# ThomasHelfer/multimodal-supernovae

Measured on AMD Instinct MI355X. Metric: contrastive pairs/sec (image+light-curve) at global batch 1024, 1/2/4/8 GPUs, higher is better.
Workload: dtype f32; 1 GPU; ViT-S/8 image tower (64x64x3, build-defined) + reference light-curve transformer (T=200, emb 64, 8 heads, depth 5, 2 bands) -> enc_dim 128, symmetric InfoNCE with all-gathered global negatives, RAdam; full train step; per_gpu_batch=1024, global_batch=1024, parallelism=dp1, launch=eager, gemm_precision=bf16x6

## Files before the change

### include/msn_hip.h

```cpp
#ifndef MSN_HIP_H
#define MSN_HIP_H

#include <stddef.h>
#include <stdint.h>

#ifdef __cplusplus
extern "C" {
#endif

#define MSN_OK 0
#define MSN_ERR_SHAPE 1
#define MSN_ERR_HIP 2

typedef void* msn_stream_t;

int msn_version(void);
const char* msn_last_error(void);
int msn_clock_probe(unsigned long long* out2, int microseconds, msn_stream_t stream);
int msn_device_count(void);

#define MSN_OP_N 0
#define MSN_OP_T 1
#define MSN_EPI_NONE 0
#define MSN_EPI_RELU 1
// ... 100 lines not shown

size_t msn_plane_bytes(int64_t R, int64_t C, int planes);
size_t msn_plane_split_colsum_workspace_bytes(int64_t R, int64_t C);
int msn_plane_split(const float* x, int64_t ldx, int64_t R, int64_t C, int planes, int transposed, void* out, float* colsum,
                    void* ws, size_t ws_bytes, msn_stream_t stream);
typedef struct msn_split_item {
    const float* x;
    int64_t ldx, R, C;
    int transposed;
    void* out;
} msn_split_item;
int msn_plane_split_list(int n, const msn_split_item* items, int planes, msn_stream_t stream);
int msn_plane_merge(const void* planes_in, int planes, int64_t R, int64_t C, float* y, int64_t ldy, msn_stream_t stream);
size_t msn_pgemm_nt_colsum_workspace_bytes(int64_t M, int N);
size_t msn_pgemm_nt_workspace_bytes(int64_t M, int N, int K, int planes, int c_planes, int epilogue, int want_colsum);
int msn_set_pgemm_tail_split(int enabled);
int msn_pgemm_nt(int64_t M, int N, int K, int planes, const void* A, const void* B, void* C, int64_t ldc, int c_planes,
                 const float* bias, int epilogue, float* aux, int64_t ldaux, float* colsum_out, void* ws, size_t ws_bytes,
                 msn_stream_t stream);
size_t msn_pgemm_tn_workspace_bytes(int64_t M, int N, int K, int planes);
int msn_pgemm_tn(int64_t M, int N, int K, int planes, const void* A, const void* B, float* C, int64_t ldc, void* ws,
                 size_t ws_bytes, msn_stream_t stream);
int msn_layernorm_fwd_planes(const float* x, int64_t ldx, int64_t rows, int cols, const float* gamma, const float* beta,
                             float eps, int planes, void* y_planes, float* y, int64_t ldy, float* mean, float* rstd,
                             msn_stream_t stream);
int msn_layernorm_bwd_planes(const float* dy, int64_t lddy, const float* x, int64_t ldx, int64_t rows, int cols,
                             const float* mean, const float* rstd, const float* gamma, const float* add, int64_t ldadd,
                             float* dx, int64_t lddx, int planes, void* dx_planes, float* dgamma, float* dbeta,
                             float* dx_colsum, void* ws, size_t ws_bytes, msn_stream_t stream);
int msn_attention_fwd_planes(const float* qkv, int64_t ldqkv, const uint8_t* key_mask, int B, int H, int T, int head_dim,
                             float scale, float* out, int64_t ldo, float* lse, int planes, void* out_planes, msn_stream_t stream);
// ... 204 lines not shown
```

### multimodal_supernovae_amd/_lib.py

```python
import ctypes
import os

import torch

_HERE = os.path.dirname(os.path.abspath(__file__))
LIB_PATH = os.environ.get("MSN_HIP_LIB") or os.path.join(_HERE, "lib", "libmsn_hip.so")

c_i64 = ctypes.c_int64
c_int = ctypes.c_int
c_f32 = ctypes.c_float
c_f64 = ctypes.c_double
c_ptr = ctypes.c_void_p
c_size = ctypes.c_size_t

SIGNATURES = {
    "msn_version": (c_int, []),
    "msn_last_error": (ctypes.c_char_p, []),
    "msn_clock_probe": (c_int, [c_ptr, c_int, c_ptr]),
    "msn_ffn_supported": (c_int, [c_i64, c_int, c_int]),
    "msn_ffn_fwd": (c_int, [c_ptr, c_i64, c_i64, c_int, c_int, c_ptr, c_ptr, c_ptr, c_ptr, c_ptr, c_i64, c_ptr]),
    "msn_ffn_bwd_workspace_bytes": (c_size, [c_i64, c_int, c_int]),
    "msn_ffn_bwd": (c_int, [c_ptr, c_i64, c_ptr, c_i64, c_i64, c_int, c_int, c_ptr, c_ptr, c_ptr, c_ptr, c_i64, c_ptr, c_ptr, c_ptr,
                            c_ptr, c_ptr, c_size, c_ptr]),
    "msn_cls_attention_supported": (c_int, [c_int, c_int]),
# ... 33 lines not shown
    "msn_masked_pool_bwd": (c_int, [c_ptr, c_ptr, c_i64, c_int, c_int, c_int, c_ptr, c_ptr, c_ptr, c_ptr]),
    "msn_mask_tokens": (c_int, [c_ptr, c_ptr, c_i64, c_int, c_ptr, c_ptr]),
    "msn_add_rows": (c_int, [c_ptr, c_i64, c_ptr, c_i64, c_i64, c_int, c_ptr]),
    "msn_plane_bytes": (c_size, [c_i64, c_i64, c_int]),
    "msn_plane_split_colsum_workspace_bytes": (c_size, [c_i64, c_i64]),
    "msn_plane_split": (c_int, [c_ptr, c_i64, c_i64, c_i64, c_int, c_int, c_ptr, c_ptr, c_ptr, c_size, c_ptr]),
    "msn_plane_split_list": (c_int, [c_int, c_ptr, c_int, c_ptr]),
    "msn_plane_split_f16": (c_int, [c_ptr, c_i64, c_i64, c_i64, c_int, c_ptr, c_ptr, c_int, c_ptr, c_ptr, c_size, c_ptr]),
    "msn_pgemm_nt_f16": (c_int, [c_i64, c_int, c_int, c_ptr, c_ptr, c_ptr, c_ptr, c_ptr, c_i64, c_ptr, c_int, c_ptr, c_i64, c_ptr,
                                 c_ptr, c_size, c_ptr]),
    "msn_pgemm_tn_f16": (c_int, [c_i64, c_int, c_int, c_ptr, c_ptr, c_ptr, c_ptr, c_ptr, c_i64, c_ptr, c_size, c_ptr]),
    "msn_plane_merge": (c_int, [c_ptr, c_int, c_i64, c_i64, c_ptr, c_i64, c_ptr]),
    "msn_pgemm_nt_colsum_workspace_bytes": (c_size, [c_i64, c_int]),
    "msn_pgemm_nt_workspace_bytes": (c_size, [c_i64, c_int, c_int, c_int, c_int, c_int, c_int]),
    "msn_set_pgemm_tail_split": (c_int, [c_int]),
    "msn_pgemm_nt": (c_int, [c_i64, c_int, c_int, c_int, c_ptr, c_ptr, c_ptr, c_i64, c_int, c_ptr, c_int, c_ptr, c_i64, c_ptr,
                             c_ptr, c_size, c_ptr]),
    "msn_pgemm_tn_workspace_bytes": (c_size, [c_i64, c_int, c_int, c_int]),
    "msn_pgemm_tn": (c_int, [c_i64, c_int, c_int, c_int, c_ptr, c_ptr, c_ptr, c_i64, c_ptr, c_size, c_ptr]),
    "msn_layernorm_fwd_planes": (c_int, [c_ptr, c_i64, c_i64, c_int, c_ptr, c_ptr, c_f32, c_int, c_ptr, c_ptr, c_i64, c_ptr, c_ptr,
                                         c_ptr]),
    "msn_layernorm_bwd_planes": (c_int, [c_ptr, c_i64, c_ptr, c_i64, c_i64, c_int, c_ptr, c_ptr, c_ptr, c_ptr, c_i64, c_ptr,
                                         c_i64, c_int, c_ptr, c_ptr, c_ptr, c_ptr, c_ptr, c_size, c_ptr]),
    "msn_bgemm_nt": (c_int, [c_i64, c_int, c_int, c_ptr, c_i64, c_ptr, c_i64, c_ptr, c_i64, c_int, c_ptr, c_int, c_ptr, c_i64,
                             c_ptr, c_ptr, c_size, c_ptr]),
    "msn_bgemm_nt_colsum_workspace_bytes": (c_size, [c_i64, c_int]),
    "msn_bgemm_tn_workspace_bytes": (c_size, [c_i64, c_int, c_int]),
    "msn_bgemm_tn": (c_int, [c_i64, c_int, c_int, c_ptr, c_i64, c_ptr, c_i64, c_ptr, c_i64, c_ptr, c_size, c_ptr]),
    "msn_cast_bf16": (c_int, [c_ptr, c_i64, c_ptr, c_ptr]),
    "msn_attention_bf16_fwd": (c_int, [c_ptr, c_i64, c_int, c_int, c_int, c_f32, c_ptr, c_i64, c_ptr, c_ptr]),
# ... 119 lines not shown
            fn.restype = res
            fn.argtypes = args
        _lib = handle
    return _lib


def require_gpu():
    if not torch.cuda.is_available():
        raise MsnHipError("multimodal_supernovae_amd needs an MI355X (gfx950): torch.cuda.is_available() is "
                          "False and the hot path has no CPU implementation")


def check(rc, what=""):
    if rc != 0:
        msg = lib().msn_last_error().decode("utf-8", "replace")
        if rc == 2 and torch.cuda.is_available() and what.startswith(("msn_sgemm", "msn_wgrad", "msn_conv2d")):
            try:
                lib().msn_reset_gemm_counters(stream_ptr())
            except Exception:
                pass
        raise MsnHipError(f"{what or 'libmsn_hip'} failed (code {rc}): {msg}")


def stream_ptr():
    return ctypes.c_void_p(torch.cuda.current_stream().cuda_stream)


def ptr(t):
    return ctypes.c_void_p(t.data_ptr()) if t is not None else ctypes.c_void_p(0)
```

### multimodal_supernovae_amd/csrc/pgemm.hip

```cpp


#include "pgemm_kernels.h"

namespace msn {
extern template __global__ void pgemm_nt_kernel<2, 128, true, false, 2, 4, false>(const PgemmArgs);
extern template __global__ void pgemm_nt_kernel<2, 128, false, false, 2, 4, false>(const PgemmArgs);
extern template __global__ void pgemm_nt_kernel<2, 128, false, true, 4, 2, false, true>(const PgemmArgs);
extern template __global__ void pgemm_tn_kernel<2, 128, true, false, 2, 4>(const PgemmArgs);
extern template __global__ void pgemm_tn_kernel<2, 128, false, false, 2, 4>(const PgemmArgs);
extern template __global__ void pgemm_tn_kernel<2, 128, true, true, 2, 4, true>(const PgemmArgs);
extern template __global__ void pgemm_tn_kernel<2, 128, false, true, 2, 4, true>(const PgemmArgs);
}

namespace msn {

__global__ __launch_bounds__(256) void pgemm_tail_finish_kernel(const PgemmArgs p, int bn) {
    const int tiles_tail = p.tiles_m * p.tiles_n - p.tail_full;
    const int per_tile = BM * bn / 4;
    const int64_t i = (int64_t)blockIdx.x * 256 + threadIdx.x;
    if (i >= (int64_t)tiles_tail * per_tile) return;
    const int tt = (int)(i / per_tile), e = (int)(i % per_tile);
    int tm, tn;
    nt_locate(p, p.tail_full + tt, tm, tn);
    const int row = e / (bn / 4), c4 = e % (bn / 4);
    const int64_t m = (int64_t)tm * BM + row;
    const int n = tn * bn + 4 * c4;
    if (m >= p.M || n >= p.N) return;
    float4 s = make_float4(0.f, 0.f, 0.f, 0.f);
    for (int g = 0; g < p.tail_segs; ++g) {
        const float4 v = *reinterpret_cast<const float4*>(p.tail_slabs + ((int64_t)(tt * p.tail_segs + g) * BM + row) * bn + 4 * c4);
        s.x += v.x; s.y += v.y; s.z += v.z; s.w += v.w;
    }
    if (p.bias) {
        const float4 b = *reinterpret_cast<const float4*>(p.bias + n);
        s.x += b.x; s.y += b.y; s.z += b.z; s.w += b.w;
    }
    if (p.epi == MSN_EPI_ADD) {
        const float4 a = *reinterpret_cast<const float4*>(p.aux + m * p.ldaux + n);
        s.x += a.x; s.y += a.y; s.z += a.z; s.w += a.w;
    } else if (p.epi == MSN_EPI_RELU) {
        s.x = fmaxf(s.x, 0.f); s.y = fmaxf(s.y, 0.f); s.z = fmaxf(s.z, 0.f); s.w = fmaxf(s.w, 0.f);
    }
    *reinterpret_cast<float4*>(static_cast<float*>(p.C) + m * p.ldc + n) = s;
}

__global__ void slab_sum_kernel(const float* __restrict__ slabs, int splits, int64_t n4, int K4, int64_t ldc4,
                                      float* __restrict__ C) {
    for (int64_t i = (int64_t)blockIdx.x * blockDim.x + threadIdx.x; i < n4; i += (int64_t)gridDim.x * blockDim.x) {
        float4 s = make_float4(0.f, 0.f, 0.f, 0.f);
        for (int k0 = 0; k0 < splits; k0 += 8) {
// ... 372 lines not shown
extern "C" int msn_plane_merge(const void* planes_in, int planes, int64_t R, int64_t C, float* y, int64_t ldy, msn_stream_t stream) {
    MSN_REQUIRE(planes_in && y && R > 0 && C > 0 && ldy >= C && planes >= 1 && planes <= 3, "msn_plane_merge: bad operand");
    const int64_t n = R * C;
    hipLaunchKernelGGL(plane_merge_kernel, dim3((unsigned)std::min<int64_t>(cdiv(n, 256), 8192)), dim3(256), 0,
                       static_cast<hipStream_t>(stream), static_cast<const unsigned char*>(planes_in), planes, R, (int)C,
                       2 * (int)cdiv(C, 32), y, ldy);
    MSN_LAUNCH_CHECK();
    return MSN_OK;
}

extern "C" size_t msn_pgemm_nt_colsum_workspace_bytes(int64_t M, int N) {
    if (M <= 0 || N <= 0) return 0;
    return sizeof(float) * (4 * (size_t)cdiv(M, BM) + COLSUM_SLICES) * (size_t)N;
}

namespace {
struct NtTail { int full, segs, steps; };
static int g_pgemm_tail = 1;
NtTail nt_tail_plan(int64_t M, int N, int K, int c_planes, int epilogue, bool want_colsum) {
    NtTail t = {0, 0, 0};
    if (!g_pgemm_tail || c_planes || want_colsum) return t;
    if (epilogue != MSN_EPI_NONE && epilogue != MSN_EPI_RELU && epilogue != MSN_EPI_ADD) return t;
    const int total = (int)(cdiv(M, BM) * cdiv(N, 128)), G = 256;
    const int nk = 2 * (int)cdiv(K, 32);
    if (total <= G / 2) {
        if (nk < 24) return t;
        int segs = std::min(std::min(G / total, nk / 4), 8);
        if (segs < 2) return t;
        t.steps = 2 * (int)cdiv(nk, 2 * segs);
        t.segs = (int)cdiv(nk, t.steps);
        t.full = 0;
        if (t.segs < 2) t = {0, 0, 0};
        return t;
    }
    if (total <= G) return t;
    const int left = total % G;
    if (left == 0 || left > G / 2 || nk < 48) return t;
    int segs = std::min(std::min(G / left, nk / 2), 16);
    if (segs < 2) return t;
    t.steps = 2 * (int)cdiv(nk, 2 * segs);
    t.segs = (int)cdiv(nk, t.steps);
    t.full = total - left;
    if (t.segs < 2) t = {0, 0, 0};
    return t;
}
}
extern "C" int msn_set_pgemm_tail_split(int enabled) {
    g_pgemm_tail = enabled ? 1 : 0;
    return MSN_OK;
}

extern "C" size_t msn_pgemm_nt_workspace_bytes(int64_t M, int N, int K, int planes, int c_planes, int epilogue, int want_colsum) {
    if (M <= 0 || N <= 0 || K <= 0) return 0;
    if (want_colsum) return std::max(msn_pgemm_nt_colsum_workspace_bytes(M, N), msn_colsum_workspace_bytes(M, N));
    const NtTail t = nt_tail_plan(M, N, K, c_planes, epilogue, false);
    const int total = (int)(cdiv(M, BM) * cdiv(N, 128));
    return t.segs ? sizeof(float) * (size_t)(total - t.full) * t.segs * BM * 128 : 0;
}

template <int NP, int BN, bool DUAL, int WM = 2, int WN = 4, bool STAG = false>
static void launch_nt(const PgemmArgs& a, bool outp, int grid, hipStream_t st) {
    if (outp) hipLaunchKernelGGL((pgemm_nt_kernel<NP, BN, true, DUAL, WM, WN, STAG>), dim3((unsigned)grid), dim3(64 * WM * WN), 0, st, a);
    else hipLaunchKernelGGL((pgemm_nt_kernel<NP, BN, false, DUAL, WM, WN, STAG>), dim3((unsigned)grid), dim3(64 * WM * WN), 0, st, a);
}

static int pgemm_nt_impl(int64_t M, int N, int K, int planes, const void* A, const void* B, void* C, int64_t ldc,
                         int c_planes, const float* bias, int epilogue, float* aux, int64_t ldaux, float* colsum_out,
                         void* ws, size_t ws_bytes, msn_stream_t stream, const float* scaleA, const float* scaleB) {
    const bool f16 = scaleA != nullptr;
    MSN_REQUIRE(M > 0 && N > 0 && K > 0 && A && B && C, "msn_pgemm_nt: empty operand");
    MSN_REQUIRE(!f16 || (scaleB && planes == 2 && !c_planes), "msn_pgemm_nt_f16: two fp16 planes per operand, both scales, fp32 result");
    MSN_REQUIRE(planes == 2 || planes == 3, "msn_pgemm_nt: planes must be 2 or 3 (got %d)", planes);
// ... 14 lines not shown
    a.cbA = a.cbB = 2 * (int)cdiv(K, 32);
    a.cbC = 2 * (int)cdiv(N, 32);
    a.epi = epilogue;
    const int bn = 128;
    a.tiles_m = (int)cdiv(M, BM); a.tiles_n = (int)cdiv(N, bn);
    a.super_rows = (int)std::max<int64_t>(1, std::min<int64_t>(8, (2 << 20) / ((int64_t)BM * K * 2 * planes)));
    a.chunk_steps = 0;
    {
        const int cs = 32;
        if ((planes == 3 || f16) && !c_planes && a.cbA > std::max(cs, 48)) {
            const int nch = (int)cdiv(a.cbA, cs);
            a.chunk_steps = 2 * (int)cdiv(a.cbA, 2 * nch);
        }
    }
    a.scaleA = scaleA, a.scaleB = scaleB;
    const NtTail tail = nt_tail_plan(M, N, K, c_planes, epilogue, colsum_out != nullptr);
    if (tail.segs && ws && ws_bytes >= msn_pgemm_nt_workspace_bytes(M, N, K, planes, c_planes, epilogue, 0) && aligned16(ws)) {
        a.tail_full = tail.full; a.tail_segs = tail.segs; a.tail_steps = tail.steps;
        a.tail_slabs = static_cast<float*>(ws);
    }
    a.colpart = nullptr;
    const bool colsum_after = colsum_out && a.chunk_steps > 0;
    if (colsum_out && !colsum_after) {
        const size_t need = msn_pgemm_nt_colsum_workspace_bytes(M, N);
        MSN_REQUIRE(ws && ws_bytes >= need && aligned16(ws), "msn_pgemm_nt: column-sum workspace %zu < %zu bytes", ws_bytes, need);
        a.colpart = static_cast<float*>(ws);
    }
    const int total = a.tiles_m * a.tiles_n;
    const int grid = a.tail_segs ? std::max(a.tail_full ? 256 : 0, (total - a.tail_full) * a.tail_segs) : std::min(total, 256);
    hipStream_t st = static_cast<hipStream_t>(stream);
    if (planes == 3) {
        a.colsum_rows = 4;
        launch_nt<3, 128, true, 4, 2>(a, c_planes != 0, grid, st);
    } else if (f16) {
        a.colsum_rows = 4;
        hipLaunchKernelGGL((pgemm_nt_kernel<2, 128, false, true, 4, 2, false, true>), dim3((unsigned)grid), dim3(512), 0, st, a);
    } else {
        launch_nt<2, 128, false>(a, c_planes != 0, grid, st);
    }
    MSN_LAUNCH_CHECK();
    if (a.tail_segs) {
        const int64_t threads = (int64_t)(total - a.tail_full) * (BM * bn / 4);
        hipLaunchKernelGGL(pgemm_tail_finish_kernel, dim3((unsigned)cdiv(threads, 256)), dim3(256), 0, st, a, bn);
        MSN_LAUNCH_CHECK();
    }
    if (colsum_after) return msn_colsum(static_cast<const float*>(C), ldc, M, N, colsum_out, ws, ws_bytes, stream);
    if (colsum_out) {
        if (colsum_finish(a.colpart, (a.colsum_rows ? a.colsum_rows : 2) * a.tiles_m, N, colsum_out, st) != MSN_OK) {
            set_error("msn_pgemm_nt: column-sum launch failed");
            return MSN_ERR_HIP;
        }
    }
    return MSN_OK;
}

extern "C" int msn_pgemm_nt(int64_t M, int N, int K, int planes, const void* A, const void* B, void* C, int64_t ldc,
                            int c_planes, const float* bias, int epilogue, float* aux, int64_t ldaux, float* colsum_out,
                            void* ws, size_t ws_bytes, msn_stream_t stream) {
// ... 90 lines not shown
```

### multimodal_supernovae_amd/csrc/pgemm_kernels.h

```cpp
#pragma once
#include <algorithm>
#include <type_traits>
#include "msn_common.h"

namespace msn {

typedef _Float16 f16x8 __attribute__((ext_vector_type(8)));
typedef unsigned u32x4 __attribute__((ext_vector_type(4)));
typedef unsigned u32x2 __attribute__((ext_vector_type(2)));
typedef __attribute__((address_space(1))) const void gptr_t;
typedef __attribute__((address_space(3))) void lptr_t;

#ifndef MSN_PG_ST_AUX
#define MSN_PG_ST_AUX 0
#endif
constexpr int BM = 256;

struct PgemmArgs {
    const unsigned char* A;
    const unsigned char* B;
    void* C;
    float* aux;
    const float* bias;
    int64_t ldc, ldaux;
    int64_t M;
    int N, K;
    int rbA, rbB;
    int cbA, cbB;
    int cbC;
    int tiles_m, tiles_n, super_rows, epi;
    int colsum_rows;
    int chunk_steps;
    int tail_full;
    int tail_segs, tail_steps;
    float* tail_slabs;
    float* colpart;
    int splits;
    int rb_per_split;
    float* slabs;
    const float* scaleA;
    const float* scaleB;
};

template <int I, int N, class F>
__device__ __forceinline__ void static_for(F&& f) {
    if constexpr (I < N) {
        f(std::integral_constant<int, I>{});
        static_for<I + 1, N>(f);
    }
}
// ... 300 lines not shown
        wait_lgkm<0>();
        wait_vm(p_was_live ? (NSLOT - 3) * ppw + (STAG ? ppw : Q_BEFORE) : 0);
#ifndef MSN_ABL_PG_NOBAR
        __builtin_amdgcn_s_barrier();
#endif
        __builtin_amdgcn_sched_barrier(0);
        if (!last) req_first(fa[(QA + NP) & 1], fb0[PAR ^ 1], nxt);
        __builtin_amdgcn_sched_barrier(0);
        mult(fa[(QA + NP - 1) & 1], fb0[PAR], SML{});
        issue_chunk(std::integral_constant<int, NG - 1>{});
        __builtin_amdgcn_sched_barrier(0);
        advance();
        c_slot = n_slot;
    };

    int eln = lane;
    int frow_e = 0, fhalf_e = 0, srow = 0, schunk = 0;
    unsigned stg = 0, st_mem = 0;
    auto epi_lane = [&]() {
        asm volatile("" : "+v"(eln));
        frow_e = eln & 31, fhalf_e = eln >> 5;
        srow = eln >> 3, schunk = eln & 7;
        stg = lds0 + (unsigned)(NSLOT * SLOT + wave * STG);
        st_mem = stg + (unsigned)(srow * 128 + ((schunk ^ srow) * 16));
    };
    auto erow = [&](int) { return frow_e; };
    auto ecolq = [&](int b) { return 2 * b + fhalf_e; };
    auto acc_addr = [&](int b) { return stg + (unsigned)(erow(b) * 128 + ((ecolq(b) ^ (erow(b) & 7)) * 16)); };
    auto lds_w128 = [&](unsigned addr, const float (&v)[4]) {
        asm volatile("ds_write_b128 %0, %1\n\ts_nop 1" ::"v"(addr), "v"(*reinterpret_cast<const f32x4*>(v)) : "memory");
// ... 26 lines not shown
    };
    auto stage_chunk = [&](int b, const float (&w)[4]) { lds_w128(acc_addr(b), w); };
    auto tile_flush = [&](rsrc_t rs, int64_t ld, int r0, int n0, auto final_) {
        constexpr int AUX = decltype(final_)::value ? MSN_PG_ST_AUX : 0;
        f32x4 r[4];
#pragma unroll
        for (int q = 0; q < 4; ++q) lds_r128(r[q], st_mem + q * 1024);
        asm volatile("s_waitcnt lgkmcnt(0)" : "+v"(r[0]), "+v"(r[1]), "+v"(r[2]), "+v"(r[3])::"memory");
        __builtin_amdgcn_sched_barrier(0);
        const int n = n0 + 4 * schunk;
        const unsigned lo = n < p.N ? (unsigned)((srow * (int)ld + n) * 4) : OOB;
#pragma unroll
        for (int q = 0; q < 4; ++q)
            __builtin_amdgcn_raw_buffer_store_b128(__builtin_bit_cast(u32x4, r[q]), rs, (int)(lo + (unsigned)((r0 + 8 * q) * (int)ld * 4)), 0, AUX);
    };
    auto slab_flush = [&](rsrc_t rs, int r0, int c0) {
        f32x4 r[4];
#pragma unroll
        for (int q = 0; q < 4; ++q) lds_r128(r[q], st_mem + q * 1024);
        asm volatile("s_waitcnt lgkmcnt(0)" : "+v"(r[0]), "+v"(r[1]), "+v"(r[2]), "+v"(r[3])::"memory");
        __builtin_amdgcn_sched_barrier(0);
#pragma unroll
        for (int q = 0; q < 4; ++q)
            __builtin_amdgcn_raw_buffer_store_b128(__builtin_bit_cast(u32x4, r[q]), rs, ((r0 + 8 * q + srow) * BN + c0 + 4 * schunk) * 4, 0, 0);
    };
    auto store_tile_epi = [&](int tm, int tn, auto epi_, auto mode_) {
        constexpr int epi = decltype(epi_)::value;
        constexpr int MODE = decltype(mode_)::value & 3;
        constexpr bool CS = (decltype(mode_)::value & 4) != 0;
        constexpr bool SLAB = (decltype(mode_)::value & 8) != 0;
        constexpr bool PARTIAL = MODE >= 2, ADDC = (MODE == 1 || MODE == 3) && !OUTP;
        constexpr bool AUXIN = !PARTIAL && (epi == MSN_EPI_RELU_BWD || epi == MSN_EPI_GELU_BWD || epi == MSN_EPI_ADD);
        epi_lane();
        if constexpr (DUAL) {
#pragma unroll
            for (int i = 0; i < MT; ++i)
#pragma unroll
                for (int j = 0; j < NT; ++j) acc[i][j] += acc2[i][j];
        }
        if constexpr (F16) {
            const float os = p.scaleA[0] * p.scaleB[0];
#pragma unroll
            for (int i = 0; i < MT; ++i)
#pragma unroll
                for (int j = 0; j < NT; ++j) acc[i][j] *= os;
        }
        constexpr bool PRE = ADDC || AUXIN;
        constexpr int PW = (MT * NT < 2) ? MT * NT : ((DUAL && !OUTP) ? MT * NT : 1);
        f32x4 pre[PRE ? PW : 1][4];
        const rsrc_t rsC = OUTP ? uniform_rsrc(static_cast<unsigned char*>(p.C) + (int64_t)tm * ARB * p.cbC * (NP * PBLK),
                                               min(max(p.rbA - tm * ARB, 0), ARB) * (int64_t)p.cbC * (NP * PBLK))
                                : rows_rsrc(static_cast<const float*>(p.C), p.ldc, tm);
        const rsrc_t rsAux = rows_rsrc(p.aux, p.ldaux, tm);
        const rsrc_t rsBias = uniform_rsrc(p.bias, p.bias ? p.N * 4 : 0);
        const rsrc_t pre_rs = ADDC ? rsC : rsAux;
        const int64_t pre_ld = ADDC ? p.ldc : p.ldaux;
// ... 2 lines not shown
            if constexpr (PRE && t < MT * NT)
                tile_fetch(pre_rs, pre_ld, wm * (32 * MT) + 32 * (t % MT), tn * BN + wn * (32 * NT) + 32 * (t / MT), pre[t % PW]);
        };
        static_for<0, PW>([&](auto t_) { pre_fetch(t_); });
        static_for<0, NT>([&](auto j_) {
            constexpr int j = decltype(j_)::value;
            const int n0 = tn * BN + wn * (32 * NT) + 32 * j;
            float cs[CS ? 16 : 1];
#pragma unroll
            for (int e = 0; e < (CS ? 16 : 1); ++e) cs[e] = 0.f;
            static_for<0, MT>([&](auto i_) {
                constexpr int i = decltype(i_)::value;
                constexpr int t = j * MT + i;
                const int64_t m0 = (int64_t)tm * BM + wm * (32 * MT) + 32 * i;
                const int rbk = tm * ARB + wm * MT + i;
                const bool live = SLAB || (n0 < p.N && (OUTP ? rbk < p.rbA : m0 < p.M));
                if (!live) {
                    pre_fetch(std::integral_constant<int, t + PW>{});
                    return;
                }
                const bool row_ok = m0 + frow_e < p.M;
                float v[16];
#pragma unroll
                for (int e = 0; e < 16; ++e) v[e] = acc[i][j][e];
                if constexpr (ADDC) {
                    float c0[16];
                    tile_take(pre[t % PW], c0);
                    pre_fetch(std::integral_constant<int, t + PW>{});
#pragma unroll
                    for (int e = 0; e < 16; ++e) v[e] += c0[e];
                }
// ... 79 lines not shown
#ifndef MSN_ABL_PG_NOPSTORE
#pragma unroll
                    for (int q = 0; q < 2 * NP; ++q)
                        if (n0 + 16 * (q / NP) < 16 * p.cbC)
                            __builtin_amdgcn_raw_buffer_store_b128(__builtin_bit_cast(u32x4, img[q]), rsC, blk + q * PBLK, 0, MSN_PG_ST_AUX);
#else
                    asm volatile("" ::"v"(img[0]), "v"(img[1]), "v"(img[2]), "v"(img[3]));
                    (void)blk;
#endif
                } else {
#pragma unroll
                    for (int b = 0; b < 4; ++b) {
                        const float w[4] = {v[4 * b], v[4 * b + 1], v[4 * b + 2], v[4 * b + 3]};
                        stage_chunk(b, w);
                    }
                    if constexpr (SLAB)
                        slab_flush(uniform_rsrc(p.tail_slabs + (int64_t)blockIdx.x * (BM * BN), BM * BN * 4), wm * (32 * MT) + 32 * i,
                                   wn * (32 * NT) + 32 * j);
                    else
                        tile_flush(rsC, p.ldc, wm * (32 * MT) + 32 * i, n0, std::integral_constant<bool, !PARTIAL>{});
                }
                if constexpr (CS) {
#pragma unroll
                    for (int e = 0; e < 16; ++e) cs[e] += v[e];
                }
            });
            if constexpr (CS) {
#pragma unroll
                for (int e = 0; e < 16; ++e) {
                    float t = cs[e];
#pragma unroll
                    for (int o = 1; o < 32; o <<= 1) t += __shfl_xor(t, o, 64);
                    cs[e] = t;
                }
                if (frow_e == 0) {
#pragma unroll
                    for (int b = 0; b < 4; ++b) {
                        const int n = n0 + 8 * b + 4 * fhalf_e;
                        if (n < p.N)
                            *reinterpret_cast<float4*>(p.colpart + (int64_t)(WM * tm + wm) * p.N + n) =
                                make_float4(cs[4 * b], cs[4 * b + 1], cs[4 * b + 2], cs[4 * b + 3]);
                    }
                }
            }
        });
    };
    auto store_tile = [&](int tm, int tn, auto mode_) {
        switch (p.epi) {
            case MSN_EPI_RELU: store_tile_epi(tm, tn, std::integral_constant<int, MSN_EPI_RELU>{}, mode_); break;
            case MSN_EPI_GELU: store_tile_epi(tm, tn, std::integral_constant<int, MSN_EPI_GELU>{}, mode_); break;
            case MSN_EPI_RELU_BWD: store_tile_epi(tm, tn, std::integral_constant<int, MSN_EPI_RELU_BWD>{}, mode_); break;
            case MSN_EPI_GELU_BWD: store_tile_epi(tm, tn, std::integral_constant<int, MSN_EPI_GELU_BWD>{}, mode_); break;
            case MSN_EPI_ADD: store_tile_epi(tm, tn, std::integral_constant<int, MSN_EPI_ADD>{}, mode_); break;
            default: store_tile_epi(tm, tn, std::integral_constant<int, MSN_EPI_NONE>{}, mode_); break;
        }
    };
    auto zero_acc = [&]() {
#pragma unroll
        for (int i = 0; i < MT; ++i)
#pragma unroll
            for (int j = 0; j < NT; ++j)
#pragma unroll
                for (int e = 0; e < 16; ++e) {
                    acc[i][j][e] = 0.f;
                    if constexpr (DUAL) acc2[i][j][e] = 0.f;
                }
    };

#pragma unroll
    for (int s = 0; s < NSLOT - 1; ++s) {
        if (p_live) {
#pragma unroll
            for (int q = 0; q < MAXQ; ++q) issue_q(q);
        }
        advance();
    }
    asm volatile("s_waitcnt vmcnt(0)" ::: "memory");
    __builtin_amdgcn_s_barrier();
    __builtin_amdgcn_sched_barrier(0);
    req_first_settled(0u);

    using T0 = std::integral_constant<int, 0>;
    using T1 = std::integral_constant<int, 1>;
    int tm, tn;
    const int csteps = (!OUTP && p.chunk_steps > 0) ? p.chunk_steps : nk;
    int kb, ke;
    for (int idx = 0; seg_of(idx, tm, tn, kb, ke); ++idx) {
        zero_acc();
        if (ke - kb < nk) {
            for (int k = kb; k < ke; k += 2) {
                step(T0{});
                step(T1{}, k + 2 >= ke);
            }
            wait_lgkm<0>();
            store_tile_epi(tm, tn, std::integral_constant<int, MSN_EPI_NONE>{}, std::integral_constant<int, 2 + 8>{});
            req_first_settled((unsigned)(c_slot * SLOT));
            continue;
        }
        int k0 = 0;
        for (; k0 + csteps < nk; k0 += csteps) {
            for (int k = 0; k < csteps; k += 2) {
                step(T0{});
                step(T1{}, k + 2 >= csteps);
            }
            wait_lgkm<0>();
            if (k0 == 0) store_tile_epi(tm, tn, std::integral_constant<int, MSN_EPI_NONE>{}, std::integral_constant<int, 2>{});
            else store_tile_epi(tm, tn, std::integral_constant<int, MSN_EPI_NONE>{}, std::integral_constant<int, 3>{});
            zero_acc();
            req_first_settled((unsigned)(c_slot * SLOT));
        }
        for (int k = k0; k < nk; k += 2) {
            step(T0{});
            step(T1{}, k + 2 >= nk);
        }
        wait_lgkm<0>();
        if (k0 != 0) store_tile(tm, tn, std::integral_constant<int, 1>{});
        else if (p.colpart) store_tile(tm, tn, std::integral_constant<int, 4>{});
        else store_tile(tm, tn, std::integral_constant<int, 0>{});
        req_first_settled((unsigned)(c_slot * SLOT));
    }
}

template <int NP, int BQ, bool SWAP, bool DUAL, int WM = 2, int WN = 4, bool F16 = false, int FOLDN = 1>
__global__ __launch_bounds__(512, 2) void pgemm_tn_kernel(const PgemmArgs p) {
    static_assert(WM * WN == 8, "eight waves");
    constexpr int PHB = 16 * NP, QHB = (BQ / 16) * NP;
    constexpr int PIECES = (PHB + QHB) / 2;
    constexpr int PP = PHB / 2;
    constexpr int SLOT = PIECES * PBLK;
    constexpr int NSLOT = (4 * SLOT <= 160 * 1024) ? 4 : 3;
    constexpr int MAXQ = (PIECES + 7) / 8;
    constexpr int MT = 8 / WM, NT = BQ / (32 * WN);
    constexpr int NG = NP * (NP + 1) / 2;
    __shared__ __attribute__((aligned(1024))) unsigned char lds[NSLOT * SLOT];
// ... 298 lines not shown
```

### multimodal_supernovae_amd/ops.py

```python
import ctypes
import os

import torch

from . import _lib
from ._lib import check, lib, ptr, stream_ptr

GEMM_PROFILE = None
ATTN_PROFILE = None

PREC_F32, PREC_BF16X3, PREC_BF16 = 0, 1, 2
PREC_PLANES3, PREC_PLANES2 = 3, 4
_PREC_NAMES = {"f32": PREC_F32, "bf16x3": PREC_BF16X3, "bf16": PREC_BF16, "bf16x6": PREC_PLANES3, "bf16x3p": PREC_PLANES2}
_C_PRECISION = {PREC_F32: PREC_F32, PREC_BF16X3: PREC_BF16X3, PREC_BF16: PREC_BF16, PREC_PLANES3: PREC_F32,
                PREC_PLANES2: PREC_BF16X3}


def plane_count(precision=None):
    p = GEMM_PRECISION if precision is None else precision
    return 3 if p == PREC_PLANES3 else 2 if p == PREC_PLANES2 else 0
GEMM_PRECISION = _PREC_NAMES[os.environ.get("MSN_GEMM_PRECISION", "bf16x6").lower()]


class gemm_precision:
# ... 1094 lines not shown
        else:
            check(L.msn_pgemm_tn(M, N, K, dy.planes, ptr(dy.buf), ptr(x.buf), ptr(c), K, ptr(ws), nb, stream_ptr()), "msn_pgemm_tn")
    return c


def layernorm_fwd_planes(x, gamma, beta, eps, planes):
    return _layernorm_fwd(x, gamma, beta, eps, planes=planes)


def layernorm_bwd_planes(dy, x, mean, rstd, gamma, planes, add=None, want_colsum=False):
    out = _layernorm_bwd(dy, x, mean, rstd, gamma, add, want_colsum, planes=planes)
    return out if want_colsum else out[:4]


def set_pgemm_tail_split(enabled):
    check(lib().msn_set_pgemm_tail_split(int(bool(enabled))))
```

Measured before the change: 15610 pairs/s.

## Finish split-K tail tiles in-kernel via atomic arrival counters and widen tail eligibility

```diff
diff --git a/include/msn_hip.h b/include/msn_hip.h
--- a/include/msn_hip.h
+++ b/include/msn_hip.h
@@ -138,7 +138,9 @@
 int msn_plane_merge(const void* planes_in, int planes, int64_t R, int64_t C, float* y, int64_t ldy, msn_stream_t stream);
 size_t msn_pgemm_nt_colsum_workspace_bytes(int64_t M, int N);
 size_t msn_pgemm_nt_workspace_bytes(int64_t M, int N, int K, int planes, int c_planes, int epilogue, int want_colsum);
-int msn_set_pgemm_tail_split(int enabled);
+int msn_set_pgemm_tail_split(int mode);
+int msn_set_pgemm_tail_plan(int max_segs, int min_steps);
+int msn_pgemm_nt_tail_plan(int64_t M, int N, int K, int planes, int c_planes, int epilogue, int want_colsum, int* out3);
 int msn_pgemm_nt(int64_t M, int N, int K, int planes, const void* A, const void* B, void* C, int64_t ldc, int c_planes,
                  const float* bias, int epilogue, float* aux, int64_t ldaux, float* colsum_out, void* ws, size_t ws_bytes,
                  msn_stream_t stream);
diff --git a/multimodal_supernovae_amd/_lib.py b/multimodal_supernovae_amd/_lib.py
--- a/multimodal_supernovae_amd/_lib.py
+++ b/multimodal_supernovae_amd/_lib.py
@@ -71,6 +71,8 @@
     "msn_pgemm_nt_colsum_workspace_bytes": (c_size, [c_i64, c_int]),
     "msn_pgemm_nt_workspace_bytes": (c_size, [c_i64, c_int, c_int, c_int, c_int, c_int, c_int]),
     "msn_set_pgemm_tail_split": (c_int, [c_int]),
+    "msn_set_pgemm_tail_plan": (c_int, [c_int, c_int]),
+    "msn_pgemm_nt_tail_plan": (c_int, [c_i64, c_int, c_int, c_int, c_int, c_int, c_int, c_ptr]),
     "msn_pgemm_nt": (c_int, [c_i64, c_int, c_int, c_int, c_ptr, c_ptr, c_ptr, c_i64, c_int, c_ptr, c_int, c_ptr, c_i64, c_ptr,
                              c_ptr, c_size, c_ptr]),
     "msn_pgemm_tn_workspace_bytes": (c_size, [c_i64, c_int, c_int, c_int]),
@@ -220,7 +222,7 @@
 def check(rc, what=""):
     if rc != 0:
         msg = lib().msn_last_error().decode("utf-8", "replace")
-        if rc == 2 and torch.cuda.is_available() and what.startswith(("msn_sgemm", "msn_wgrad", "msn_conv2d")):
+        if rc == 2 and torch.cuda.is_available() and what.startswith(("msn_sgemm", "msn_wgrad", "msn_conv2d", "msn_pgemm_nt")):
             try:
                 lib().msn_reset_gemm_counters(stream_ptr())
             except Exception:
diff --git a/multimodal_supernovae_amd/csrc/pgemm.hip b/multimodal_supernovae_amd/csrc/pgemm.hip
--- a/multimodal_supernovae_amd/csrc/pgemm.hip
+++ b/multimodal_supernovae_amd/csrc/pgemm.hip
@@ -14,7 +14,7 @@
 
 namespace msn {
 
-__global__ __launch_bounds__(256) void pgemm_tail_finish_kernel(const PgemmArgs p, int bn) {
+__global__ __launch_bounds__(256) void pgemm_tail_finish_kernel(const PgemmArgs p, int bn, int wm_) {
     const int tiles_tail = p.tiles_m * p.tiles_n - p.tail_full;
     const int per_tile = BM * bn / 4;
     const int64_t i = (int64_t)blockIdx.x * 256 + threadIdx.x;
@@ -22,18 +22,21 @@
     const int tt = (int)(i / per_tile), e = (int)(i % per_tile);
     int tm, tn;
     nt_locate(p, p.tail_full + tt, tm, tn);
-    const int row = e / (bn / 4), c4 = e % (bn / 4);
+    const int wn_ = 8 / wm_, mt = 8 / wm_, nt = bn / (32 * wn_);
+    const int lane = e & 63, b = (e >> 6) & 3, q = (e >> 8) % (mt * nt), wave = (e >> 8) / (mt * nt);
+    const int row = (wave / wn_) * (32 * mt) + 32 * (q % mt) + (lane & 31);
+    const int col = (wave % wn_) * (32 * nt) + 32 * (q / mt) + 8 * b + 4 * (lane >> 5);
     const int64_t m = (int64_t)tm * BM + row;
-    const int n = tn * bn + 4 * c4;
+    const int n = tn * bn + col;
     if (m >= p.M || n >= p.N) return;
     float4 s = make_float4(0.f, 0.f, 0.f, 0.f);
     for (int g = 0; g < p.tail_segs; ++g) {
-        const float4 v = *reinterpret_cast<const float4*>(p.tail_slabs + ((int64_t)(tt * p.tail_segs + g) * BM + row) * bn + 4 * c4);
+        const float4 v = *reinterpret_cast<const float4*>(p.tail_slabs + (int64_t)(tt * p.tail_segs + g) * (BM * bn) + 4 * e);
         s.x += v.x; s.y += v.y; s.z += v.z; s.w += v.w;
     }
     if (p.bias) {
-        const float4 b = *reinterpret_cast<const float4*>(p.bias + n);
-        s.x += b.x; s.y += b.y; s.z += b.z; s.w += b.w;
+        const float4 b4 = *reinterpret_cast<const float4*>(p.bias + n);
+        s.x += b4.x; s.y += b4.y; s.z += b4.z; s.w += b4.w;
     }
     if (p.epi == MSN_EPI_ADD) {
         const float4 a = *reinterpret_cast<const float4*>(p.aux + m * p.ldaux + n);
@@ -436,13 +439,24 @@
     return sizeof(float) * (4 * (size_t)cdiv(M, BM) + COLSUM_SLICES) * (size_t)N;
 }
 
+namespace msn {
+unsigned* gemm_counter_slice(hipStream_t st);
+}
 namespace {
 struct NtTail { int full, segs, steps; };
-static int g_pgemm_tail = 1;
+static int g_pgemm_tail = 3;
+static int g_tail_max_segs = 0;
+static int g_tail_min_steps = 0;
+constexpr int TAIL_SHORT_MAX_SEGS = 6, TAIL_SHORT_MIN_STEPS = 4, TAIL_SHORT_MIN_NK = 24;
+constexpr int TAIL_ARRIVER_MAX_TILES = 32;
+bool tail_launch_form(int c_planes, int epilogue, bool want_colsum) {
+    return !c_planes && !want_colsum && (epilogue == MSN_EPI_NONE || epilogue == MSN_EPI_RELU || epilogue == MSN_EPI_ADD);
+}
 NtTail nt_tail_plan(int64_t M, int N, int K, int c_planes, int epilogue, bool want_colsum) {
     NtTail t = {0, 0, 0};
-    if (!g_pgemm_tail || c_planes || want_colsum) return t;
-    if (epilogue != MSN_EPI_NONE && epilogue != MSN_EPI_RELU && epilogue != MSN_EPI_ADD) return t;
+    if (!g_pgemm_tail) return t;
+    const bool launch_form = tail_launch_form(c_planes, epilogue, want_colsum);
+    if (g_pgemm_tail == 2 && !launch_form) return t;
     const int total = (int)(cdiv(M, BM) * cdiv(N, 128)), G = 256;
     const int nk = 2 * (int)cdiv(K, 32);
     if (total <= G / 2) {
@@ -457,8 +471,13 @@
     }
     if (total <= G) return t;
     const int left = total % G;
-    if (left == 0 || left > G / 2 || nk < 48) return t;
-    int segs = std::min(std::min(G / left, nk / 2), 16);
+    if (left == 0 || left > G / 2) return t;
+    if (!launch_form && left > TAIL_ARRIVER_MAX_TILES && g_tail_max_segs == 0) return t;
+    const bool long_k = nk >= 48;
+    const int max_segs = g_tail_max_segs > 0 ? g_tail_max_segs : (long_k ? 16 : TAIL_SHORT_MAX_SEGS);
+    const int min_steps = std::max(2, g_tail_min_steps > 0 ? g_tail_min_steps : (long_k ? 2 : TAIL_SHORT_MIN_STEPS));
+    if (!long_k && nk < TAIL_SHORT_MIN_NK && g_tail_max_segs == 0) return t;
+    int segs = std::min(std::min(G / left, nk / min_steps), max_segs);
     if (segs < 2) return t;
     t.steps = 2 * (int)cdiv(nk, 2 * segs);
     t.segs = (int)cdiv(nk, t.steps);
@@ -466,18 +485,39 @@
     if (t.segs < 2) t = {0, 0, 0};
     return t;
 }
+size_t nt_colsum_ws_bytes(int64_t M, int N) {
+    const size_t b = std::max(msn_pgemm_nt_colsum_workspace_bytes(M, N), msn_colsum_workspace_bytes(M, N));
+    return (b + 255) / 256 * 256;
+}
+size_t nt_slab_bytes(int64_t M, int N, const NtTail& t) {
+    const int total = (int)(cdiv(M, BM) * cdiv(N, 128));
+    return t.segs ? sizeof(float) * (size_t)(total - t.full) * t.segs * BM * 128 : 0;
+}
 }
 extern "C" int msn_set_pgemm_tail_split(int enabled) {
-    g_pgemm_tail = enabled ? 1 : 0;
+    MSN_REQUIRE(enabled >= 0 && enabled <= 3, "msn_set_pgemm_tail_split: 0 (off), 1 (in-kernel finish), 2 (finishing launch) or 3 (the faster of the two per launch)");
+    g_pgemm_tail = enabled;
+    return MSN_OK;
+}
+extern "C" int msn_set_pgemm_tail_plan(int max_segs, int min_steps) {
+    MSN_REQUIRE(max_segs >= 0 && max_segs <= 16 && min_steps >= 0, "msn_set_pgemm_tail_plan: 0 - 16 segments, min_steps >= 0 (0 = the built-in rule)");
+    g_tail_max_segs = max_segs, g_tail_min_steps = min_steps;
+    return MSN_OK;
+}
+extern "C" int msn_pgemm_nt_tail_plan(int64_t M, int N, int K, int planes, int c_planes, int epilogue, int want_colsum, int* out3) {
+    MSN_REQUIRE(out3 && M > 0 && N > 0 && K > 0, "msn_pgemm_nt_tail_plan: bad argument");
+    (void)planes;
+    const NtTail t = nt_tail_plan(M, N, K, c_planes, epilogue, want_colsum != 0);
+    out3[0] = t.segs ? t.full : (int)(cdiv(M, BM) * cdiv(N, 128)), out3[1] = t.segs, out3[2] = t.steps;
     return MSN_OK;
 }
 
 extern "C" size_t msn_pgemm_nt_workspace_bytes(int64_t M, int N, int K, int planes, int c_planes, int epilogue, int want_colsum) {
     if (M <= 0 || N <= 0 || K <= 0) return 0;
-    if (want_colsum) return std::max(msn_pgemm_nt_colsum_workspace_bytes(M, N), msn_colsum_workspace_bytes(M, N));
-    const NtTail t = nt_tail_plan(M, N, K, c_planes, epilogue, false);
-    const int total = (int)(cdiv(M, BM) * cdiv(N, 128));
-    return t.segs ? sizeof(float) * (size_t)(total - t.full) * t.segs * BM * 128 : 0;
+    (void)planes;
+    const size_t slabs = nt_slab_bytes(M, N, nt_tail_plan(M, N, K, c_planes, epilogue, want_colsum != 0));
+    if (!want_colsum) return slabs;
+    return slabs ? nt_colsum_ws_bytes(M, N) + slabs : std::max(msn_pgemm_nt_colsum_workspace_bytes(M, N), msn_colsum_workspace_bytes(M, N));
 }
 
 template <int NP, int BN, bool DUAL, int WM = 2, int WN = 4, bool STAG = false>
@@ -522,10 +562,17 @@
         }
     }
     a.scaleA = scaleA, a.scaleB = scaleB;
+    hipStream_t st = static_cast<hipStream_t>(stream);
     const NtTail tail = nt_tail_plan(M, N, K, c_planes, epilogue, colsum_out != nullptr);
-    if (tail.segs && ws && ws_bytes >= msn_pgemm_nt_workspace_bytes(M, N, K, planes, c_planes, epilogue, 0) && aligned16(ws)) {
-        a.tail_full = tail.full; a.tail_segs = tail.segs; a.tail_steps = tail.steps;
-        a.tail_slabs = static_cast<float*>(ws);
+    if (tail.segs && ws && aligned16(ws)) {
+        const size_t off = colsum_out ? nt_colsum_ws_bytes(M, N) : 0;
+        const bool simple = tail_launch_form(c_planes, epilogue, colsum_out != nullptr);
+        unsigned* counters = (g_pgemm_tail == 1 || (g_pgemm_tail == 3 && !simple)) ? gemm_counter_slice(st) : nullptr;
+        if (ws_bytes >= off + nt_slab_bytes(M, N, tail) && (counters || simple)) {
+            a.tail_full = tail.full; a.tail_segs = tail.segs; a.tail_steps = tail.steps;
+            a.tail_slabs = reinterpret_cast<float*>(static_cast<unsigned char*>(ws) + off);
+            a.tail_counter = counters;
+        }
     }
     a.colpart = nullptr;
     const bool colsum_after = colsum_out && a.chunk_steps > 0;
@@ -536,7 +583,6 @@
     }
     const int total = a.tiles_m * a.tiles_n;
     const int grid = a.tail_segs ? std::max(a.tail_full ? 256 : 0, (total - a.tail_full) * a.tail_segs) : std::min(total, 256);
-    hipStream_t st = static_cast<hipStream_t>(stream);
     if (planes == 3) {
         a.colsum_rows = 4;
         launch_nt<3, 128, true, 4, 2>(a, c_planes != 0, grid, st);
@@ -547,9 +593,9 @@
         launch_nt<2, 128, false>(a, c_planes != 0, grid, st);
     }
     MSN_LAUNCH_CHECK();
-    if (a.tail_segs) {
+    if (a.tail_segs && !a.tail_counter) {
         const int64_t threads = (int64_t)(total - a.tail_full) * (BM * bn / 4);
-        hipLaunchKernelGGL(pgemm_tail_finish_kernel, dim3((unsigned)cdiv(threads, 256)), dim3(256), 0, st, a, bn);
+        hipLaunchKernelGGL(pgemm_tail_finish_kernel, dim3((unsigned)cdiv(threads, 256)), dim3(256), 0, st, a, bn, (planes == 3 || f16) ? 4 : 2);
         MSN_LAUNCH_CHECK();
     }
     if (colsum_after) return msn_colsum(static_cast<const float*>(C), ldc, M, N, colsum_out, ws, ws_bytes, stream);
diff --git a/multimodal_supernovae_amd/csrc/pgemm_kernels.h b/multimodal_supernovae_amd/csrc/pgemm_kernels.h
--- a/multimodal_supernovae_amd/csrc/pgemm_kernels.h
+++ b/multimodal_supernovae_amd/csrc/pgemm_kernels.h
@@ -34,6 +34,7 @@
     int tail_full;
     int tail_segs, tail_steps;
     float* tail_slabs;
+    unsigned* tail_counter;
     float* colpart;
     int splits;
     int rb_per_split;
@@ -364,6 +365,7 @@
         c_slot = n_slot;
     };
 
+    bool sums_final = false;
     int eln = lane;
     int frow_e = 0, fhalf_e = 0, srow = 0, schunk = 0;
     unsigned stg = 0, st_mem = 0;
@@ -420,32 +422,23 @@
         for (int q = 0; q < 4; ++q)
             __builtin_amdgcn_raw_buffer_store_b128(__builtin_bit_cast(u32x4, r[q]), rs, (int)(lo + (unsigned)((r0 + 8 * q) * (int)ld * 4)), 0, AUX);
     };
-    auto slab_flush = [&](rsrc_t rs, int r0, int c0) {
-        f32x4 r[4];
-#pragma unroll
-        for (int q = 0; q < 4; ++q) lds_r128(r[q], st_mem + q * 1024);
-        asm volatile("s_waitcnt lgkmcnt(0)" : "+v"(r[0]), "+v"(r[1]), "+v"(r[2]), "+v"(r[3])::"memory");
-        __builtin_amdgcn_sched_barrier(0);
-#pragma unroll
-        for (int q = 0; q < 4; ++q)
-            __builtin_amdgcn_raw_buffer_store_b128(__builtin_bit_cast(u32x4, r[q]), rs, ((r0 + 8 * q + srow) * BN + c0 + 4 * schunk) * 4, 0, 0);
-    };
-    auto store_tile_epi = [&](int tm, int tn, auto epi_, auto mode_) {
+    auto store_tile_epi = [&](int tm, int tn, auto epi_, auto mode_) __attribute__((always_inline)) {
         constexpr int epi = decltype(epi_)::value;
         constexpr int MODE = decltype(mode_)::value & 3;
         constexpr bool CS = (decltype(mode_)::value & 4) != 0;
-        constexpr bool SLAB = (decltype(mode_)::value & 8) != 0;
         constexpr bool PARTIAL = MODE >= 2, ADDC = (MODE == 1 || MODE == 3) && !OUTP;
         constexpr bool AUXIN = !PARTIAL && (epi == MSN_EPI_RELU_BWD || epi == MSN_EPI_GELU_BWD || epi == MSN_EPI_ADD);
         epi_lane();
         if constexpr (DUAL) {
-#pragma unroll
-            for (int i = 0; i < MT; ++i)
-#pragma unroll
-                for (int j = 0; j < NT; ++j) acc[i][j] += acc2[i][j];
+            if (!sums_final) {
+#pragma unroll
+                for (int i = 0; i < MT; ++i)
+#pragma unroll
+                    for (int j = 0; j < NT; ++j) acc[i][j] += acc2[i][j];
+            }
         }
         if constexpr (F16) {
-            const float os = p.scaleA[0] * p.scaleB[0];
+            const float os = sums_final ? 1.f : p.scaleA[0] * p.scaleB[0];
 #pragma unroll
             for (int i = 0; i < MT; ++i)
 #pragma unroll
@@ -478,7 +471,7 @@
                 constexpr int t = j * MT + i;
                 const int64_t m0 = (int64_t)tm * BM + wm * (32 * MT) + 32 * i;
                 const int rbk = tm * ARB + wm * MT + i;
-                const bool live = SLAB || (n0 < p.N && (OUTP ? rbk < p.rbA : m0 < p.M));
+                const bool live = n0 < p.N && (OUTP ? rbk < p.rbA : m0 < p.M);
                 if (!live) {
                     pre_fetch(std::integral_constant<int, t + PW>{});
                     return;
@@ -588,11 +581,7 @@
                         const float w[4] = {v[4 * b], v[4 * b + 1], v[4 * b + 2], v[4 * b + 3]};
                         stage_chunk(b, w);
                     }
-                    if constexpr (SLAB)
-                        slab_flush(uniform_rsrc(p.tail_slabs + (int64_t)blockIdx.x * (BM * BN), BM * BN * 4), wm * (32 * MT) + 32 * i,
-                                   wn * (32 * NT) + 32 * j);
-                    else
-                        tile_flush(rsC, p.ldc, wm * (32 * MT) + 32 * i, n0, std::integral_constant<bool, !PARTIAL>{});
+                    tile_flush(rsC, p.ldc, wm * (32 * MT) + 32 * i, n0, std::integral_constant<bool, !PARTIAL>{});
                 }
                 if constexpr (CS) {
 #pragma unroll
@@ -619,7 +608,7 @@
             }
         });
     };
-    auto store_tile = [&](int tm, int tn, auto mode_) {
+    auto store_tile = [&](int tm, int tn, auto mode_) __attribute__((always_inline)) {
         switch (p.epi) {
             case MSN_EPI_RELU: store_tile_epi(tm, tn, std::integral_constant<int, MSN_EPI_RELU>{}, mode_); break;
             case MSN_EPI_GELU: store_tile_epi(tm, tn, std::integral_constant<int, MSN_EPI_GELU>{}, mode_); break;
@@ -641,6 +630,44 @@
                 }
     };
 
+    constexpr int SC1 = 16;
+    auto slab_rsrc = [&](int slab) { return uniform_rsrc(p.tail_slabs + (int64_t)slab * (BM * BN), BM * BN * 4); };
+    auto slab_lane = [&]() {
+        asm volatile("" : "+v"(eln));
+        return (wave * (MT * NT * 4) * 64 + eln) * 16;
+    };
+    auto slab_store = [&]() {
+        const rsrc_t rs = slab_rsrc((int)blockIdx.x);
+        const int off = slab_lane();
+        float os = 1.f;
+        if constexpr (F16) os = p.scaleA[0] * p.scaleB[0];
+        static_for<0, MT * NT>([&](auto q_) {
+            constexpr int q = decltype(q_)::value;
+            f32x16 v = acc[q % MT][q / MT];
+            if constexpr (DUAL) v += acc2[q % MT][q / MT];
+            if constexpr (F16) v *= os;
+#pragma unroll
+            for (int b = 0; b < 4; ++b) {
+                const f32x4 w = {v[4 * b], v[4 * b + 1], v[4 * b + 2], v[4 * b + 3]};
+                __builtin_amdgcn_raw_buffer_store_b128(__builtin_bit_cast(u32x4, w), rs, off, (q * 4 + b) * 1024, SC1);
+            }
+        });
+    };
+    constexpr int TT = MT * NT;
+    typedef f32x4 tile_regs[4];
+    auto slab_fetch = [&](int slab, int off, auto q_, tile_regs& t) {
+        constexpr int q = decltype(q_)::value;
+        const rsrc_t rs = slab_rsrc(slab);
+#pragma unroll
+        for (int b = 0; b < 4; ++b)
+            t[b] = __builtin_bit_cast(f32x4, __builtin_amdgcn_raw_buffer_load_b128(rs, off, (q * 4 + b) * 1024, SC1));
+    };
+    auto slab_add = [&](auto q_, const tile_regs& t) {
+        constexpr int q = decltype(q_)::value;
+#pragma unroll
+        for (int e = 0; e < 16; ++e) acc[q % MT][q / MT][e] += t[e / 4][e % 4];
+    };
+
 #pragma unroll
     for (int s = 0; s < NSLOT - 1; ++s) {
         if (p_live) {
@@ -659,6 +686,7 @@
     int tm, tn;
     const int csteps = (!OUTP && p.chunk_steps > 0) ? p.chunk_steps : nk;
     int kb, ke;
+    bool finisher = false;
     for (int idx = 0; seg_of(idx, tm, tn, kb, ke); ++idx) {
         zero_acc();
         if (ke - kb < nk) {
@@ -667,9 +695,22 @@
                 step(T1{}, k + 2 >= ke);
             }
             wait_lgkm<0>();
-            store_tile_epi(tm, tn, std::integral_constant<int, MSN_EPI_NONE>{}, std::integral_constant<int, 2 + 8>{});
-            req_first_settled((unsigned)(c_slot * SLOT));
-            continue;
+            slab_store();
+            if (p.tail_counter) {
+                asm volatile("s_waitcnt vmcnt(0)" ::: "memory");
+                __syncthreads();
+                unsigned* flag = reinterpret_cast<unsigned*>(lds);
+                if (threadIdx.x == 0) {
+                    unsigned* cnt = p.tail_counter + (int)blockIdx.x / p.tail_segs;
+                    const unsigned prev = __hip_atomic_fetch_add(cnt, 1u, __ATOMIC_RELAXED, __HIP_MEMORY_SCOPE_AGENT);
+                    const unsigned last = prev + 1u == (unsigned)p.tail_segs ? 1u : 0u;
+                    if (last) __hip_atomic_store(cnt, 0u, __ATOMIC_RELAXED, __HIP_MEMORY_SCOPE_AGENT);
+                    *flag = last;
+                }
+                __syncthreads();
+                finisher = __builtin_amdgcn_readfirstlane((int)*flag) != 0;
+            }
+            break;
         }
         int k0 = 0;
         for (; k0 + csteps < nk; k0 += csteps) {
@@ -692,6 +733,41 @@
         else if (p.colpart) store_tile(tm, tn, std::integral_constant<int, 4>{});
         else store_tile(tm, tn, std::integral_constant<int, 0>{});
         req_first_settled((unsigned)(c_slot * SLOT));
+    }
+    if (finisher) {
+        const int first = ((int)blockIdx.x / p.tail_segs) * p.tail_segs, S = p.tail_segs;
+#pragma unroll
+        for (int i = 0; i < MT; ++i)
+#pragma unroll
+            for (int j = 0; j < NT; ++j)
+#pragma unroll
+                for (int e = 0; e < 16; ++e) acc[i][j][e] = 0.f;
+        const int off = slab_lane();
+        tile_regs A[TT], B[TT - 1];
+        using LAST = std::integral_constant<int, TT - 1>;
+        static_for<0, TT>([&](auto q_) { slab_fetch(first, off, q_, A[decltype(q_)::value]); });
+        for (int s = 0; s < S; s += 2) {
+            const bool odd = s + 1 < S, next = s + 2 < S;
+            if (odd) static_for<0, TT - 1>([&](auto q_) { slab_fetch(first + s + 1, off, q_, B[decltype(q_)::value]); });
+            __builtin_amdgcn_sched_barrier(0);
+            slab_add(LAST{}, A[TT - 1]);
+            __builtin_amdgcn_sched_barrier(0);
+            if (odd) slab_fetch(first + s + 1, off, LAST{}, A[TT - 1]);
+            __builtin_amdgcn_sched_barrier(0);
+            static_for<0, TT - 1>([&](auto q_) { slab_add(q_, A[decltype(q_)::value]); });
+            __builtin_amdgcn_sched_barrier(0);
+            if (next) static_for<0, TT - 1>([&](auto q_) { slab_fetch(first + s + 2, off, q_, A[decltype(q_)::value]); });
+            __builtin_amdgcn_sched_barrier(0);
+            if (odd) {
+                static_for<0, TT - 1>([&](auto q_) { slab_add(q_, B[decltype(q_)::value]); });
+                slab_add(LAST{}, A[TT - 1]);
+            }
+            __builtin_amdgcn_sched_barrier(0);
+            if (next) slab_fetch(first + s + 2, off, LAST{}, A[TT - 1]);
+        }
+        sums_final = true;
+        if (p.colpart) store_tile(tm, tn, std::integral_constant<int, 4>{});
+        else store_tile(tm, tn, std::integral_constant<int, 0>{});
     }
 }
 
diff --git a/multimodal_supernovae_amd/ops.py b/multimodal_supernovae_amd/ops.py
--- a/multimodal_supernovae_amd/ops.py
+++ b/multimodal_supernovae_amd/ops.py
@@ -1132,4 +1132,15 @@
 
 
 def set_pgemm_tail_split(enabled):
-    check(lib().msn_set_pgemm_tail_split(int(bool(enabled))))
+    check(lib().msn_set_pgemm_tail_split((3 if enabled else 0) if isinstance(enabled, bool) else int(enabled)))
+
+
+def set_pgemm_tail_plan(max_segs=0, min_steps=0):
+    check(lib().msn_set_pgemm_tail_plan(int(max_segs), int(min_steps)))
+
+
+def pgemm_tail_plan(M, N, K, planes=3, out_planes=False, epilogue=EPI_NONE, want_colsum=False):
+    out = (ctypes.c_int * 3)()
+    check(lib().msn_pgemm_nt_tail_plan(M, N, K, planes, 1 if out_planes else 0, epilogue, 1 if want_colsum else 0,
+                                       ctypes.cast(out, ctypes.c_void_p)), "msn_pgemm_nt_tail_plan")
+    return tuple(out)
```

Result: no change. 15670 pairs/s, median of 6 (+0.4%).
